# OpenDriveLab/kai0

Measured on AMD Instinct MI355X. Metric: train samples/sec pi0.5 full FT, higher is better.
Workload: dtype bf16; 1 GPU; pi0.5 full fine-tune bf16, batch 32 per MI355X, 3-cam 224x224 (BASELINE.json configs[1]); global_batch=32, seq_len=1018, parallelism=dp1

## Files before the change

### kai0_amd/csrc/gemm_bf16.hip

```cpp
#include "common.h"
#include "../../include/kai0hip.h"
#include <stdlib.h>
#include <algorithm>
#include <atomic>
#include <type_traits>

namespace {

constexpr int BK = 64;

#ifdef KAI0_ABLATE
#define KAI0_ABL(p) ((p).ablate)
#else
#define KAI0_ABL(p) 0
#endif

struct RowMap {
    int32_t rpb;
    int64_t bs, off;
    __device__ __forceinline__ int64_t operator()(int r) const {
        if (rpb == 0) return r;
        const int q = r / rpb;
        return (int64_t)q * bs + (r - q * rpb) + off;
    }
};

struct GemmArgs {
    const bf16_t* A;
    const bf16_t* B;
    void* C;
    int M, N, K;
    int64_t lda, ldb, ldc;
    int batch_inner;
    int64_t sA1, sA2, sB1, sB2, sC1, sC2;
    RowMap amap, bmap, cmap;
    const void* bias;
    int bias_f32;
    float scale;
    int act;
    int out_f32;
    bf16_t* pre_out;
    const bf16_t* aux1;
    const bf16_t* aux2;
    const bf16_t* gate;
    int gate_rpb;
    int accumulate;
    int64_t gate_ld;
    const bf16_t* residual;
    int64_t ldr, sR1, sR2;
    int tiles_m, tiles_n;
    int ablate;
    int nt_c;
    int simple_epi;
    int nt_pre;
    const float* rowvec;
    int64_t rv_s1, rv_s2, rv_ld;
    int nseg;
    bf16_t* seg_dst[3];
    int64_t seg_ld[3];
    int seg_begin[3];
    float* ws;
    int split_k, k_chunk;
    const bf16_t* B2;
    bf16_t* pre_out2;
    bf16_t* norm_out;
    const void* norm_w;
    const bf16_t* norm_b;
    float norm_eps;
    int norm_kind;
    const bf16_t* rope_cos;
    const bf16_t* rope_sin;
    int rope_half, rope_n_end;
};

typedef __attribute__((ext_vector_type(4))) int i32x4_t;
constexpr uint32_t OOB = 0x80000000u;
__device__ __forceinline__ void glds16(__amdgpu_buffer_rsrc_t rsrc, uint32_t voff, char* lds_dst_wave_uniform) {
    __builtin_amdgcn_raw_ptr_buffer_load_lds(rsrc, (LDS_PTR(void))lds_dst_wave_uniform, 16, (int)voff, 0, 0, 0);
}


__device__ __forceinline__ void store_pre8(bf16_t* dst, bf16x8 v, int nt) {
    if (nt) __builtin_nontemporal_store(v, reinterpret_cast<bf16x8*>(dst));
    else *reinterpret_cast<bf16x8*>(dst) = v;
}

// ... 99 lines not shown
        }
        *reinterpret_cast<f32x4*>(cp) = f32x4{v[0], v[1], v[2], v[3]};
        *reinterpret_cast<f32x4*>(cp + 4) = f32x4{v[4], v[5], v[6], v[7]};
    } else {
        bf16_t* cp = reinterpret_cast<bf16_t*>(cbase) + cz + orow * p.ldc + ccol;
        if (p.nseg > 0) {
            int si = 0;
            if (p.nseg > 1 && ccol >= p.seg_begin[1]) si = 1;
            if (p.nseg > 2 && ccol >= p.seg_begin[2]) si = 2;
            cp = p.seg_dst[si] + orow * p.seg_ld[si] + (ccol - p.seg_begin[si]);
        }
        if (p.accumulate) {
            bf16x8 ov = *reinterpret_cast<const bf16x8*>(cp);
#pragma unroll
            for (int e = 0; e < 8; ++e) v[e] += bf2f(ov[e]);
        }
        bf16x8 ov;
#pragma unroll
        for (int e = 0; e < 8; ++e) ov[e] = f2bf(v[e]);
        store_pre8(cp, ov, p.nt_c);
    }
}

#define N_ALIGNED8(n) (((n) & 7) == 0)

__device__ __forceinline__ void lds_barrier() {
    __builtin_amdgcn_sched_barrier(0);
    asm volatile("s_waitcnt lgkmcnt(0)" ::: "memory");
    __builtin_amdgcn_s_barrier();
    asm volatile("" ::: "memory");
    __builtin_amdgcn_sched_barrier(0);
}

template <bool A_KC, bool B_KC, int WM, int WN, int MT, int NT, bool PP, int NS = 2, int BKT = 64, int SCH = 0>
__global__ __launch_bounds__(WM * WN * 64, (WM * WN * 64) / 256) void gemm_bf16_kernel(const GemmArgs p) {
    static_assert(PP ? (WM == 2 && WN == 4 && MT == 8 && ((SCH == 1 && NS == 2 && BKT == 64) || (SCH == 3 && NS == 4 && BKT == 32)))
                     : (SCH == 0 && NS >= 2 && BKT == 64),
                  "K loops: plain multi-stage (SCH 0, 64 deep), quadrant (SCH 1: 256x256x64, 2 stages), ring (SCH 3: 256x256x32, 4 slots)");
    constexpr int BK = BKT;
    constexpr int NWAVES = WM * WN;
    constexpr int TBM = WM * MT * 16, TBN = WN * NT * 16;
    constexpr int A_TILE = TBM * BK * 2, B_TILE = TBN * BK * 2;
    constexpr int STAGE = A_TILE + B_TILE;
    constexpr int NA = A_TILE / 1024 / NWAVES;
    constexpr int NB = B_TILE / 1024 / NWAVES;
    constexpr int KC_CPR = BK / 8;
    constexpr int KC_RPP = 64 / KC_CPR;
    constexpr int A_ROWB = TBM * 2, B_ROWB = TBN * 2;
    constexpr int A_LPR = A_ROWB / 16, B_LPR = B_ROWB / 16;
    constexpr int A_RPP = 64 / A_LPR, B_RPP = 64 / B_LPR;
    constexpr int GROUP = TBM == 128 ? 8 : 4;
    static_assert(NA >= 1 && NB >= 1 && NT == 4 && ((MT % 4) == 0 || MT == 2), "unsupported tile configuration");
    constexpr int AH = MT >= 4 ? 4 : MT;
    static_assert(A_KC || (64 % A_LPR) == 0, "contraction-strided A needs a power-of-two tile height");
    extern __shared__ __attribute__((aligned(16))) char smem[];

    const int tid = threadIdx.x;
    const int lane = tid & 63;
    const int wave = __builtin_amdgcn_readfirstlane(tid >> 6);
    const int wm = wave / WN, wn = wave % WN;
    if constexpr (MT <= 4) {
        asm volatile("" ::"s"(p.A), "s"(p.B), "s"(p.M), "s"(p.N), "s"(p.K), "s"(p.lda), "s"(p.ldb), "s"(p.tiles_m), "s"(p.tiles_n),
                     "s"(p.split_k), "s"(p.k_chunk), "s"(p.batch_inner), "s"(p.amap.rpb), "s"(p.bmap.rpb), "s"(p.act), "s"(p.sA1),
                     "s"(p.sB1), "s"(p.sA2), "s"(p.sB2));
    }
    const int nwg = gridDim.x;
    int pid = blockIdx.x;
    {
// ... 252 lines not shown
        issue_half(false, 1, 0);
        issue_half(false, 0, 1);
        issue_half(true, 1, 1);
        asm volatile("s_waitcnt vmcnt(6)" ::: "memory");
        lds_barrier();
        if (grp == 1) lds_barrier();
        bf16x8 af[4][2], bq[2][2];
        auto read_a = [&](const char* ta, int h) {
#pragma unroll
            for (int i = 0; i < 4; ++i)
#pragma unroll
                for (int ks = 0; ks < 2; ++ks)
                    af[i][ks] = A_KC ? load_frag(ta, true, A_ROWB, wm * 128 + (h * 4 + i) * 16, ks)
                                     : load_frag(ta + h * 16384, false, 256, wm * 64 + i * 16, ks);
        };
        auto read_b = [&](const char* tb, int h) {
#pragma unroll
            for (int j = 0; j < 2; ++j)
#pragma unroll
                for (int ks = 0; ks < 2; ++ks)
                    bq[j][ks] = B_KC ? load_frag(tb, true, B_ROWB, wn * 64 + (h * 2 + j) * 16, ks)
                                     : load_frag(tb + h * 16384, false, 256, wn * 32 + j * 16, ks);
        };
        auto quad = [&](auto ahc, auto bhc) {
            constexpr int ah = decltype(ahc)::value, bh = decltype(bhc)::value;
            __builtin_amdgcn_s_setprio(1);
#pragma unroll
            for (int ks = 0; ks < 2; ++ks)
#pragma unroll
                for (int i = 0; i < 4; ++i)
#pragma unroll
                    for (int j = 0; j < 2; ++j)
                        acc[ah * 4 + i][bh * 2 + j] =
                            __builtin_amdgcn_mfma_f32_16x16x32_bf16(af[i][ks], bq[j][ks], acc[ah * 4 + i][bh * 2 + j], 0, 0, 0);
            __builtin_amdgcn_s_setprio(0);
        };
        using I0 = std::integral_constant<int, 0>;
        using I1 = std::integral_constant<int, 1>;
        for (int t = 0; t < nk; ++t) {
            const char* ta = smem + (t & 1) * STAGE;
            const char* tb = ta + A_TILE;
            read_b(tb, 0);
            __builtin_amdgcn_sched_barrier(0);
            read_a(ta, 0);
            __builtin_amdgcn_sched_barrier(0);
            issue_half(true, 0, t + 1);
            lds_barrier();
            quad(I0{}, I0{});
            lds_barrier();
            read_b(tb, 1);
            __builtin_amdgcn_sched_barrier(0);
            issue_half(false, 1, t + 1);
            asm volatile("s_waitcnt vmcnt(8)" ::: "memory");
            lds_barrier();
            quad(I0{}, I1{});
            lds_barrier();
            read_a(ta, 1);
            __builtin_amdgcn_sched_barrier(0);
            issue_half(false, 0, t + 2);
            lds_barrier();
            quad(I1{}, I1{});
            lds_barrier();
            read_b(tb, 0);
            __builtin_amdgcn_sched_barrier(0);
            issue_half(true, 1, t + 2);
            asm volatile("s_waitcnt vmcnt(6)" ::: "memory");
            lds_barrier();
            quad(I1{}, I0{});
            lds_barrier();
        }
        asm volatile("s_waitcnt vmcnt(0)" ::: "memory");
        if (grp == 0) lds_barrier();
        lds_barrier();
    } else {
#pragma unroll
        for (int st = 0; st < NS - 1; ++st)
            if (st < nk) stage(st, st);
        int slot_c = 0, slot_p = NS - 1;
        for (int kt = 0; kt < nk; ++kt) {
            if constexpr (NS == 2) {
                asm volatile("s_waitcnt vmcnt(0)" ::: "memory");
            } else {
                if (kt + NS - 2 < nk) asm volatile("s_waitcnt vmcnt(%0)" ::"n"((NS - 2) * (NA + NB)) : "memory");
                else asm volatile("s_waitcnt vmcnt(0)" ::: "memory");
            }
            lds_barrier();
            if (kt + NS - 1 < nk && KAI0_ABL(p) != 1) stage(kt + NS - 1, slot_p);
            const char* ta = smem + slot_c * STAGE;
            const char* tb = ta + A_TILE;
    #pragma unroll
            for (int ks = 0; ks < BK / 32; ++ks) {
                bf16x8 bfr[NT];
    #pragma unroll
                for (int t = 0; t < NT; ++t) bfr[t] = load_frag(tb, B_KC, B_ROWB, wn * (NT * 16) + t * 16, ks);
    #pragma unroll
                for (int h = 0; h < MT / AH; ++h) {
                    bf16x8 af[AH];
    #pragma unroll
                    for (int t = 0; t < AH; ++t) af[t] = load_frag(ta, A_KC, A_ROWB, wm * (MT * 16) + (h * AH + t) * 16, ks);
    #pragma unroll
                    for (int i = 0; i < AH; ++i)
    #pragma unroll
                        for (int j = 0; j < NT; ++j)
                            acc[h * AH + i][j] = __builtin_amdgcn_mfma_f32_16x16x32_bf16(af[i], bfr[j], acc[h * AH + i][j], 0, 0, 0);
                }
            }
            slot_c = slot_c + 1 == NS ? 0 : slot_c + 1;
            slot_p = slot_p + 1 == NS ? 0 : slot_p + 1;
        }
        lds_barrier();
    }

    float* slab = reinterpret_cast<float*>(smem + wave * (AH * 4096));
    const int64_t cz = z1 * p.sC1 + z2 * p.sC2;
    const int64_t rz = z1 * p.sR1 + z2 * p.sR2;
    const int64_t vz = z1 * p.rv_s1 + z2 * p.rv_s2;
    constexpr bool ILM = SCH == 1 && !A_KC, ILN = SCH == 1 && !B_KC;
    const int ccol = ILN ? n0 + ((lane & 7) >> 2) * 128 + wn * 32 + ((lane & 7) & 3) * 8 : n0 + wn * 64 + (lane & 7) * 8;
    auto row_base = [&](int h) { return ILM ? m0 + h * 128 + wm * 64 : m0 + wm * (MT * 16) + h * 64; };
    const bool col_ok = ccol < ((p.N + 7) & ~7);
    const bool fused_fast = p.act >= 2 && p.split_k == 1 && p.bias == nullptr && p.gate == nullptr && p.residual == nullptr &&
                            !p.accumulate && !p.out_f32 && p.nseg == 0 && (p.act == 4 || p.scale == 1.0f) &&
                            (p.act != 3 || p.pre_out != nullptr);
    const bool plain_fast = p.act <= 1 && p.split_k == 1 && (p.bias != nullptr || p.residual != nullptr) && p.gate == nullptr &&
                            !p.accumulate && !p.out_f32 && p.nseg == 0 && (N_ALIGNED8(p.N));
    const bool simple_fast = MT == 8 && p.simple_epi && p.act <= 1 && p.split_k == 1 && p.gate == nullptr && !p.out_f32 && p.scale == 1.0f &&
                             p.cmap.rpb == 0 && (N_ALIGNED8(p.N));
    auto epi_half = [&](auto hc) {
        constexpr int h = decltype(hc)::value;
        if constexpr (((MT == 4 && WM == 2) || (MT == 2 && WM == 4)) && WN == 2 && A_KC && B_KC) if (p.act == 7) {
            const bool rot = n0 < p.rope_n_end;
            const int fi = ((n0 >> 7) & 1) * 64 + (lane & 7) * 8;
            const int rcol = rot ? (n0 >> 8) * 256 + wn * 128 + fi : n0 + wn * 64 + (lane & 7) * 8;
            const int rbase = row_base(h) + (lane >> 3);
            bf16x8 cs[AH * 2], sn[AH * 2];
#pragma unroll
            for (int it = 0; it < AH * 2; ++it) {
                const int64_t tr = (int64_t)min(rbase + it * 8, p.M - 1) * p.rope_half + fi;
                cs[it] = *reinterpret_cast<const bf16x8*>(p.rope_cos + (rot ? tr : 0));
                sn[it] = *reinterpret_cast<const bf16x8*>(p.rope_sin + (rot ? tr : 0));
            }
#pragma unroll
            for (int i = 0; i < AH; ++i)
#pragma unroll
                for (int j = 0; j < 4; ++j)
#pragma unroll
                    for (int r = 0; r < 4; ++r) slab[(i * 16 + 4 * g + r) * 64 + j * 16 + l15] = acc[i][j][r];
            lds_barrier();
            const float* pslab = reinterpret_cast<const float*>(smem + (wave ^ 1) * (AH * 4096));
            int si = 0;
            if (p.nseg > 1 && rcol >= p.seg_begin[1]) si = 1;
            if (p.nseg > 2 && rcol >= p.seg_begin[2]) si = 2;
            const bool rcol_ok = rcol < p.N;
#pragma unroll
            for (int it = 0; it < AH * 2; ++it) {
                const int lr = it * 8 + (lane >> 3);
                const int row = rbase + it * 8;
                const int so = lr * 64 + (lane & 7) * 8;
                const f32x4 v0 = *reinterpret_cast<const f32x4*>(slab + so), v1 = *reinterpret_cast<const f32x4*>(slab + so + 4);
                const f32x4 w0 = *reinterpret_cast<const f32x4*>(pslab + so), w1 = *reinterpret_cast<const f32x4*>(pslab + so + 4);
// ... 334 lines not shown
            float v[8] = {v0[0], v0[1], v0[2], v0[3], v1[0], v1[1], v1[2], v1[3]};
            if (p.split_k > 1) {
                float* wp = reinterpret_cast<float*>(p.ws) + ((int64_t)blockIdx.y * p.M + row) * p.N + ccol;
                *reinterpret_cast<f32x4*>(wp) = v0;
                *reinterpret_cast<f32x4*>(wp + 4) = v1;
            } else {
                epilogue8(p, v, row, ccol, cz, rz, vz, p.C, p.out_f32 != 0);
            }
        }
        asm volatile("s_waitcnt lgkmcnt(0)" ::: "memory");
        __builtin_amdgcn_wave_barrier();
    };
    epi_half(std::integral_constant<int, 0>{});
    if constexpr (MT / 4 > 1) epi_half(std::integral_constant<int, 1>{});
    if constexpr (MT / 4 > 2) epi_half(std::integral_constant<int, 2>{});
    static_assert(MT / 4 <= 3, "extend the epilogue parts");
}

constexpr int PS_SLOTS = 1024;
__device__ unsigned int g_ps_ctr[PS_SLOTS][16];

#ifdef KAI0_PS_TRACE
__device__ long long g_ps_trace[256][8];
#define PS_STAMP(i)                                              \
    do {                                                         \
        const long long n_ = __builtin_amdgcn_s_memrealtime();   \
        t_acc[i] += n_ - t_prev;                                 \
        t_prev = n_;                                             \
    } while (0)
#else
#define PS_STAMP(i) do { } while (0)
#endif

__global__ __launch_bounds__(512, 1) void gemm_nt_persistent_kernel(const GemmArgs p, unsigned int* __restrict__ ctr) {
    constexpr int TBM = 256, TBN = 256, A_TILE = TBM * BK * 2, STAGE = 2 * A_TILE, GROUP = 4, MT = 8;
    extern __shared__ __attribute__((aligned(16))) char smem[];
    const int tid = threadIdx.x, lane = tid & 63;
    const int wave = __builtin_amdgcn_readfirstlane(tid >> 6);
    const int wm = wave >> 2, wn = wave & 3, grp = wm;
    const int l15 = lane & 15, g = lane >> 4;
    int* mbox = reinterpret_cast<int*>(smem + 2 * STAGE);
    float* slab = reinterpret_cast<float*>(smem + 2 * STAGE + wave * 4096);
    const int ntile = p.tiles_m * p.tiles_n;
    const int qq = ntile >> 3, rr = ntile & 7;
    const int x0 = blockIdx.x & 7;
    auto draw = [&]() -> unsigned { return __hip_atomic_fetch_add(ctr + x0, 1u, __ATOMIC_RELAXED, __HIP_MEMORY_SCOPE_AGENT); };
    auto resolve = [&](unsigned t) -> int {
        for (int a = 0; a < 8; ++a) {
            const int x = (x0 + a) & 7;
            const int len = qq + (x < rr ? 1 : 0);
            if (a > 0) t = __hip_atomic_fetch_add(ctr + x, 1u, __ATOMIC_RELAXED, __HIP_MEMORY_SCOPE_AGENT);
            if ((int)t < len) return (x < rr ? x * (qq + 1) : rr * (qq + 1) + (x - rr) * qq) + (int)t;
        }
        return -1;
    };
    auto next_ticket = [&]() -> int { return resolve(draw()); };
    const __amdgpu_buffer_rsrc_t a_rsrc = __builtin_amdgcn_make_buffer_rsrc((void*)p.A, 0, (int)OOB, 0x00020000);
    const __amdgpu_buffer_rsrc_t b_rsrc = __builtin_amdgcn_make_buffer_rsrc((void*)p.B, 0, (int)OOB, 0x00020000);
    const bool pair = p.act == 6;
    const __amdgpu_buffer_rsrc_t b2_rsrc = __builtin_amdgcn_make_buffer_rsrc((void*)(pair ? p.B2 : p.B), 0, (int)OOB, 0x00020000);
    const int kc_chunk = ((lane & 7) ^ (lane >> 3)) * 8;
    const int nk = (p.K + BK - 1) / BK;

    const uint32_t lda2 = (uint32_t)p.lda * 2, ldb2 = (uint32_t)p.ldb * 2, kc2 = (uint32_t)kc_chunk * 2;
    auto arow_fix = [](int) -> uint32_t { return 0u; };
    int m0 = 0, n0 = 0;
// ... 74 lines not shown
#ifdef KAI0_PS_TRACE
    long long t_acc[5] = {0, 0, 0, 0, 0};
    long long t_prev = __builtin_amdgcn_s_memrealtime();
#endif
    while (cur >= 0) {
        f32x4 acc[MT][4];
#pragma unroll
        for (int i = 0; i < MT; ++i)
#pragma unroll
            for (int j = 0; j < 4; ++j) acc[i][j] = f32x4{0.f, 0.f, 0.f, 0.f};
        bf16x8 af[4][2], bq[2][2];
        auto read_a = [&](const char* ta, int h) {
#pragma unroll
            for (int i = 0; i < 4; ++i)
#pragma unroll
                for (int ks = 0; ks < 2; ++ks) af[i][ks] = frag(ta, wm * 128 + (h * 4 + i) * 16, ks);
        };
        auto read_b = [&](const char* tb, int h) {
#pragma unroll
            for (int j = 0; j < 2; ++j)
#pragma unroll
                for (int ks = 0; ks < 2; ++ks) bq[j][ks] = frag(tb, wn * 64 + (h * 2 + j) * 16, ks);
        };
        auto quad = [&](auto ahc, auto bhc) {
            constexpr int ah = decltype(ahc)::value, bh = decltype(bhc)::value;
            __builtin_amdgcn_s_setprio(1);
#pragma unroll
            for (int ks = 0; ks < 2; ++ks)
#pragma unroll
                for (int i = 0; i < 4; ++i)
#pragma unroll
                    for (int j = 0; j < 2; ++j)
                        acc[ah * 4 + i][bh * 2 + j] =
                            __builtin_amdgcn_mfma_f32_16x16x32_bf16(af[i][ks], bq[j][ks], acc[ah * 4 + i][bh * 2 + j], 0, 0, 0);
            __builtin_amdgcn_s_setprio(0);
        };
        using I0 = std::integral_constant<int, 0>;
        using I1 = std::integral_constant<int, 1>;
        PS_STAMP(0);
        for (int t = 0; t < nk; ++t) {
            const char* ta = smem + (t & 1) * STAGE;
            const char* tb = ta + A_TILE;
            read_b(tb, 0);
            __builtin_amdgcn_sched_barrier(0);
            read_a(ta, 0);
            __builtin_amdgcn_sched_barrier(0);
            issue_half(true, 0, t + 1);
            lds_barrier();
            quad(I0{}, I0{});
            lds_barrier();
            read_b(tb, 1);
            __builtin_amdgcn_sched_barrier(0);
            issue_half(false, 1, t + 1);
            asm volatile("s_waitcnt vmcnt(8)" ::: "memory");
            lds_barrier();
            quad(I0{}, I1{});
            lds_barrier();
            read_a(ta, 1);
            __builtin_amdgcn_sched_barrier(0);
            issue_half(false, 0, t + 2);
            lds_barrier();
            quad(I1{}, I1{});
            lds_barrier();
            read_b(tb, 0);
            __builtin_amdgcn_sched_barrier(0);
            issue_half(true, 1, t + 2);
            asm volatile("s_waitcnt vmcnt(6)" ::: "memory");
            lds_barrier();
            quad(I1{}, I0{});
            lds_barrier();
        }
        asm volatile("s_waitcnt vmcnt(0)" ::: "memory");
        if (grp == 0) lds_barrier();
        lds_barrier();

        PS_STAMP(1);
        const int m0c = m0, n0c = n0;
        int nn = -1;
        unsigned raw = 0;
        if (tid == 0 && nxt >= 0) raw = draw();
        if (nxt >= 0) {
            setup(nxt);
            prologue_issue();
        }
        const int ccol = n0c + wn * 64 + (lane & 7) * 8;
        const bool col_ok = ccol < ((p.N + 7) & ~7);
        const bool fused_fast = p.act >= 2 && p.act <= 5 && p.bias == nullptr && p.gate == nullptr && p.residual == nullptr && !p.accumulate &&
                                !p.out_f32 && p.nseg == 0 && (p.act == 4 || p.scale == 1.0f) && (p.act != 3 || p.pre_out != nullptr);
        const bool simple_fast = p.simple_epi && p.act <= 1 && p.split_k == 1 && p.gate == nullptr && !p.out_f32 && p.scale == 1.0f && p.cmap.rpb == 0 &&
                                 (N_ALIGNED8(p.N));
        auto to_slab = [&](int ti) {
            __builtin_amdgcn_wave_barrier();
#pragma unroll
            for (int j = 0; j < 4; ++j)
#pragma unroll
                for (int r = 0; r < 4; ++r) slab[(4 * g + r) * 64 + j * 16 + l15] = acc[ti][j][r];
            asm volatile("s_waitcnt lgkmcnt(0)" ::: "memory");
            __builtin_amdgcn_wave_barrier();
        };
        if (pair) {
            const int ocol = (n0c >> 1) + wn * 32 + (lane & 3) * 8;
            const bool ocol_ok = ocol < (p.N >> 1);
            bf16_t* cb = reinterpret_cast<bf16_t*>(p.C);
#pragma unroll
            for (int ti = 0; ti < MT; ++ti) {
                to_slab(ti);
                const int row = m0c + wm * 128 + ti * 16 + (lane >> 2);
                const float* sp = slab + (lane >> 2) * 64 + (lane & 3) * 8;
                const f32x4 g0 = *reinterpret_cast<const f32x4*>(sp), g1 = *reinterpret_cast<const f32x4*>(sp + 4);
                const f32x4 u0 = *reinterpret_cast<const f32x4*>(sp + 32), u1 = *reinterpret_cast<const f32x4*>(sp + 36);
                if (row < p.M && ocol_ok) {
                    const float gv[8] = {g0[0], g0[1], g0[2], g0[3], g1[0], g1[1], g1[2], g1[3]};
                    const float uv[8] = {u0[0], u0[1], u0[2], u0[3], u1[0], u1[1], u1[2], u1[3]};
                    bf16x8 gb, ub, hb;
#pragma unroll
                    for (int e = 0; e < 8; e += 2) {
                        const f32x2 gr = rbf2(f32x2{gv[e], gv[e + 1]}), ur = rbf2(f32x2{uv[e], uv[e + 1]});
                        const f32x2 hv = rbf2(gelu_tanh2(gr)) * ur;
                        gb[e] = f2bf(gr[0]); gb[e + 1] = f2bf(gr[1]);
                        ub[e] = f2bf(ur[0]); ub[e + 1] = f2bf(ur[1]);
                        hb[e] = f2bf(hv[0]); hb[e + 1] = f2bf(hv[1]);
                    }
                    const int64_t o = p.cmap(row) * p.ldc + ocol;
                    *reinterpret_cast<bf16x8*>(cb + o) = hb;
                    if (p.pre_out != nullptr) store_pre8(p.pre_out + o, gb, p.nt_pre);
                    if (p.pre_out2 != nullptr) store_pre8(p.pre_out2 + o, ub, p.nt_pre);
                }
            }
        } else if (fused_fast) {
            bf16_t* cb = reinterpret_cast<bf16_t*>(p.C);
#pragma unroll
            for (int h = 0; h < 2; ++h) {
                bf16x8 s0[8], s1[8];
// ... 300 lines not shown
        float ss = 0.f;
#pragma unroll
        for (int e = 0; e < 8; ++e) ss += x[e] * x[e];
        const float rstd = rsqrtf(block_sum<4>(ss, red) / (float)p.N + p.norm_eps);
#pragma unroll
        for (int e = 0; e < 8; ++e) y[e] = (x[e] * rstd) * (1.0f + wv[e]);
    } else {
        float sm = 0.f;
#pragma unroll
        for (int e = 0; e < 8; ++e) sm += x[e];
        const float mean = block_sum<4>(sm, red) / (float)p.N;
        float vs = 0.f;
#pragma unroll
        for (int e = 0; e < 8; ++e) {
            const float d = x[e] - mean;
            vs += live ? d * d : 0.f;
        }
        const float rstd = rsqrtf(block_sum<4>(vs, red) / (float)p.N + p.norm_eps);
#pragma unroll
        for (int e = 0; e < 8; ++e) y[e] = (x[e] - mean) * rstd * wv[e] + bv[e];
    }
    if (live) {
        bf16x8 o;
#pragma unroll
        for (int e = 0; e < 8; ++e) o[e] = f2bf(y[e]);
        *reinterpret_cast<bf16x8*>(p.norm_out + (int64_t)row * p.N + col) = o;
    }
}

constexpr int layout_bit(bool a_kc, bool b_kc) { return 1 << (2 * a_kc + b_kc); }
constexpr int L_NT = layout_bit(true, true), L_NN = layout_bit(true, false), L_TT = layout_bit(false, true), L_TN = layout_bit(false, false);
constexpr int L_ALL = L_NT | L_NN | L_TT | L_TN;

template <int LAYOUTS, int WM, int WN, int MT, int NT, bool PP, int NS = 2, int BKT = 64, int SCH = 0>
int launch_cfg(const kai0_gemm_desc* d, GemmArgs& p, int batch, hipStream_t s) {
    constexpr int TBM = WM * MT * 16, TBN = WN * NT * 16;
    constexpr int LDS = NS * (TBM + TBN) * BKT * 2;
    p.tiles_m = (d->M + TBM - 1) / TBM;
    p.tiles_n = (p.N + TBN - 1) / TBN;
    dim3 grid(p.tiles_m * p.tiles_n, batch * p.split_k, 1), block(WM * WN * 64, 1, 1);
#define KAI0_LAUNCH(AK, BK_)                                                                                      \
    if constexpr ((LAYOUTS & layout_bit(AK, BK_)) != 0)                                                          \
        if ((d->a_kc != 0) == AK && (d->b_kc != 0) == BK_) {                                                      \
            static bool attr_set = false;                                                                         \
            auto kern = gemm_bf16_kernel<AK, BK_, WM, WN, MT, NT, PP, NS, BKT, SCH>;                              \
            if (!attr_set) {                                                                                      \
                hipError_t e = hipFuncSetAttribute((const void*)kern, hipFuncAttributeMaxDynamicSharedMemorySize, LDS); \
                if (e != hipSuccess) {                                                                            \
                    kai0_set_error("kai0_gemm_bf16: cannot reserve %d B of LDS: %s", LDS, hipGetErrorString(e));  \
                    return -2;                                                                                    \
                }                                                                                                 \
                attr_set = true;                                                                                  \
            }                                                                                                     \
            hipLaunchKernelGGL(kern, grid, block, LDS, s, p);                                                     \
            return 0;                                                                                             \
        }
    KAI0_LAUNCH(true, true)
    KAI0_LAUNCH(true, false)
    KAI0_LAUNCH(false, true)
    KAI0_LAUNCH(false, false)
#undef KAI0_LAUNCH
    kai0_set_error("kai0_gemm_bf16: the %d x %d tile configuration (%d waves, %d stages) is not built for a_kc=%d b_kc=%d", TBM, TBN,
                   WM * WN, NS, d->a_kc, d->b_kc);
    return -3;
}

}

#ifdef KAI0_PS_TRACE
KAI0_API int kai0_debug_ps_trace(long long* host_out) {
    return (int)hipMemcpyFromSymbol(host_out, HIP_SYMBOL(g_ps_trace), sizeof(long long) * 256 * 8);
}
#endif

KAI0_API int kai0_gemm_bf16(const kai0_gemm_desc* d, kai0_stream_t stream) {
    KAI0_REQUIRE(d != nullptr, "kai0_gemm_bf16: null descriptor");
    KAI0_REQUIRE(d->M > 0 && d->N > 0 && d->K > 0, "kai0_gemm_bf16: empty problem M=%d N=%d K=%d", d->M, d->N,
                 d->K);
    KAI0_REQUIRE(d->A && d->B && d->C, "kai0_gemm_bf16: null operand");
    KAI0_REQUIRE((d->lda % 8) == 0 && (d->ldb % 8) == 0 && (d->ldc % 8) == 0,
                 "kai0_gemm_bf16: leading dims must be multiples of 8 (lda=%lld ldb=%lld ldc=%lld)",
                 (long long)d->lda, (long long)d->ldb, (long long)d->ldc);
    KAI0_REQUIRE((d->N % 8) == 0 || (d->b_kc && d->ldc >= ((d->N + 7) & ~7) && !d->bias && !d->gate && !d->residual &&
                                     !d->pre_out && !d->accumulate),
                 "kai0_gemm_bf16: N=%d not a multiple of 8 needs b_kc, padded C rows and a plain epilogue", d->N);
    KAI0_REQUIRE((d->K % 8) == 0 || (!d->a_kc && !d->b_kc), "kai0_gemm_bf16: K=%d must be a multiple of 8 for "
                 "K-contiguous operands", d->K);
    KAI0_REQUIRE(d->a_kc || (d->M % 8) == 0, "kai0_gemm_bf16: M=%d must be a multiple of 8 when A is [K][M]",
                 d->M);
    KAI0_REQUIRE(((uintptr_t)d->A % 16) == 0 && ((uintptr_t)d->B % 16) == 0 && ((uintptr_t)d->C % 16) == 0,
                 "kai0_gemm_bf16: operands must be 16-byte aligned");
    KAI0_REQUIRE(d->batch <= 1 || (((d->sA1 | d->sA2 | d->sB1 | d->sB2) & 7) == 0 && ((d->sC1 | d->sC2) & (d->out_f32 ? 3 : 7)) == 0),
                 "kai0_gemm_bf16: batch strides must be multiples of 8 elements (16 B)");
    KAI0_REQUIRE(d->gate == nullptr || d->gate_rpb > 0, "kai0_gemm_bf16: gate needs gate_rpb > 0");
    KAI0_REQUIRE(d->act >= 0 && d->act <= 7, "kai0_gemm_bf16: unknown act %d", d->act);
    KAI0_REQUIRE(d->persist >= 0 && d->persist <= 2 && d->small_w8 >= 0 && d->small_w8 <= 2 && d->general_epilogue >= 0 &&
                     d->general_epilogue <= 1,
                 "kai0_gemm_bf16: hook out of range (persist=%d, small_w8=%d: 0..2; general_epilogue=%d: 0..1)", d->persist, d->small_w8,
                 d->general_epilogue);
    KAI0_REQUIRE(d->act != 7 || (d->rope_cos && d->rope_sin && d->rope_half == 128 && d->rope_n_end > 0 && (d->rope_n_end % 256) == 0 &&
                                 d->rope_n_end <= d->N && (d->N % 128) == 0 && d->a_kc && d->b_kc && d->batch <= 1 && d->split_k <= 1 &&
                                 !d->out_f32 && !d->accumulate && !d->bias && !d->gate && !d->residual && !d->pre_out &&
                                 (d->scale == 0.0f || d->scale == 1.0f) && d->b_rpb == 0 && ((uintptr_t)d->rope_cos % 16) == 0 &&
                                 ((uintptr_t)d->rope_sin % 16) == 0),
                 "kai0_gemm_bf16: act=7 (RoPE epilogue) needs bf16 cos / sin tables [M][128], rope_n_end %% 256 == 0, N %% 128 == 0, K-contiguous "
                 "operands, one batch entry, no split-K, a plain bf16 output");
    KAI0_REQUIRE(d->act != 6 || (d->B2 && d->a_kc && d->b_kc && d->batch <= 1 && d->split_k <= 1 && !d->out_f32 && !d->accumulate &&
                                 d->nseg == 0 && !d->bias && !d->gate && !d->residual && (d->scale == 0.0f || d->scale == 1.0f) &&
                                 (d->N % 32) == 0 && d->b_rpb == 0 && ((uintptr_t)d->B2 % 16) == 0),
                 "kai0_gemm_bf16: act=6 (GeGLU pair) needs B2 = up weight, K-contiguous operands, N %% 32 == 0, one batch entry, a "
                 "plain bf16 output");
    KAI0_REQUIRE(d->norm_kind == 0 ||
                     ((d->norm_kind == 1 || d->norm_kind == 2) && d->split_k > 1 && d->norm_out && d->norm_w && (d->norm_kind == 1 || d->norm_b) &&
                      d->batch <= 1 && !d->out_f32 && d->nseg == 0 && (d->N % 8) == 0 && d->N <= 2048 && d->act == 0 && !d->gate &&
                      !d->rowvec && ((uintptr_t)d->norm_out % 16) == 0 && ((uintptr_t)d->norm_w % 16) == 0),
                 "kai0_gemm_bf16: a fused norm (norm_kind=%d) needs split_k > 1, norm_out / norm_w (/ norm_b), one batch entry, a plain "
                 "bf16 output with N %% 8 == 0, N <= 2048, no activation / gate", d->norm_kind);
    KAI0_REQUIRE(d->act != 5 || (d->aux1 && !d->out_f32 && !d->accumulate && d->nseg == 0 && (d->N % 8) == 0),
                 "kai0_gemm_bf16: act=5 (fused GELU backward) needs aux1 = pre-activation, plain bf16 output");
    KAI0_REQUIRE(d->act != 4 || (d->aux1 && d->rowvec && !d->out_f32 && !d->accumulate && d->nseg == 0 && (d->N % 8) == 0),
                 "kai0_gemm_bf16: act=4 (fused softmax backward) needs aux1 = P, rowvec = D, plain bf16 output");
    KAI0_REQUIRE(d->act < 2 || d->act >= 4 || ((d->pre_out || d->act == 2) && d->aux1 && (d->act == 2 || d->aux2) && !d->out_f32 && (d->N % 8) == 0),
                 "kai0_gemm_bf16: act=%d (fused GeGLU) needs pre_out and aux inputs, bf16 output", d->act);
    KAI0_REQUIRE(d->nseg >= 0 && d->nseg <= 3, "kai0_gemm_bf16: nseg=%d", d->nseg);
    if (d->nseg > 0) {
        KAI0_REQUIRE(!d->out_f32 && !d->accumulate && (d->batch <= 1) && (d->act < 2 || d->act == 7) && !d->pre_out && (d->N % 8) == 0,
                     "kai0_gemm_bf16: column segments need a plain bf16 epilogue, batch 1");
        KAI0_REQUIRE(d->act != 4, "kai0_gemm_bf16: column segments and act=4 are exclusive");
        for (int i = 0; i < d->nseg; ++i)
            KAI0_REQUIRE(d->seg[i].dst && (d->seg[i].ld % 8) == 0 && (d->seg[i].n_begin % 8) == 0 &&
                             ((uintptr_t)d->seg[i].dst % 16) == 0 && d->seg[i].n_begin == (i ? d->seg[i].n_begin : 0) &&
// ... 19 lines not shown
    p.pre_out2 = (bf16_t*)d->pre_out2;
    p.norm_out = (bf16_t*)d->norm_out;
    p.norm_w = d->norm_w;
    p.norm_b = (const bf16_t*)d->norm_b;
    p.norm_eps = d->norm_eps;
    p.norm_kind = d->norm_kind;
    p.rope_cos = (const bf16_t*)d->rope_cos;
    p.rope_sin = (const bf16_t*)d->rope_sin;
    p.rope_half = d->rope_half;
    p.rope_n_end = d->rope_n_end;
    p.lda = d->lda; p.ldb = d->ldb; p.ldc = d->ldc;
    p.batch_inner = d->batch_inner > 0 ? d->batch_inner : 1;
    p.sA1 = d->sA1; p.sA2 = d->sA2; p.sB1 = d->sB1; p.sB2 = d->sB2; p.sC1 = d->sC1; p.sC2 = d->sC2;
    p.amap = RowMap{d->a_rpb, d->a_bs, d->a_off};
    p.bmap = RowMap{d->b_rpb, d->b_bs, d->b_off};
    p.cmap = RowMap{d->c_rpb, d->c_bs, d->c_off};
    p.bias = d->bias; p.bias_f32 = d->bias_f32;
    p.scale = d->scale == 0.0f ? 1.0f : d->scale;
    p.act = d->act; p.out_f32 = d->out_f32;
    p.pre_out = (bf16_t*)d->pre_out;
    p.aux1 = (const bf16_t*)d->aux1;
    p.aux2 = (const bf16_t*)d->aux2;
    p.gate = (const bf16_t*)d->gate; p.gate_rpb = d->gate_rpb; p.gate_ld = d->gate_ld;
    p.accumulate = d->accumulate;
    p.residual = (const bf16_t*)d->residual; p.ldr = d->ldr; p.sR1 = d->sR1; p.sR2 = d->sR2;
#ifdef KAI0_ABLATE
    static const int ablate = [] { const char* e = getenv("KAI0_GEMM_ABLATE"); return e ? atoi(e) : 0; }();
    p.ablate = ablate;
#else
    p.ablate = 0;
#endif
    p.nt_pre = 1;
    p.nt_c = d->c_nontemporal != 0;
    p.simple_epi = d->general_epilogue == 0;
    p.rowvec = d->rowvec; p.rv_s1 = d->rv_s1; p.rv_s2 = d->rv_s2; p.rv_ld = d->rv_ld;
    p.nseg = d->nseg;
    for (int i = 0; i < 3; ++i) {
        p.seg_dst[i] = i < d->nseg ? (bf16_t*)d->seg[i].dst : nullptr;
        p.seg_ld[i] = i < d->nseg ? d->seg[i].ld : 0;
        p.seg_begin[i] = i < d->nseg ? d->seg[i].n_begin : 0;
    }
    p.split_k = 1;
    p.k_chunk = d->K;
    const int split = d->split_k > 1 ? d->split_k : 1;
    p.ws = nullptr;
    if (split > 1) {
        KAI0_REQUIRE(d->workspace != nullptr && d->workspace_bytes >= (int64_t)batch * split * d->M * d->N * 4,
                     "kai0_gemm_bf16: split_k=%d needs a workspace of batch*split*M*N*4 bytes", split);
        KAI0_REQUIRE((d->N % 8) == 0, "kai0_gemm_bf16: split_k needs N %% 8 == 0");
        p.split_k = split;
        p.k_chunk = ((d->K + split - 1) / split + BK - 1) / BK * BK;
        p.ws = (float*)d->workspace;
    }
    const int64_t big_tiles = (int64_t)((d->M + 255) / 256) * ((p.N + 255) / 256) * batch * (split > 1 ? split : 1);
    const bool big = d->act != 7 && big_tiles >= 160 && d->K >= 256;
    hipStream_t s = (hipStream_t)stream;
    int rc;
    const int64_t small_blocks = (int64_t)((d->M + 127) / 128) * ((p.N + 127) / 128) * batch * (split > 1 ? split : 1);
    const bool deep = small_blocks <= 256 && p.k_chunk >= 256;
    const bool w8 = !big && d->a_kc && d->b_kc && (d->act <= 1 || d->act == 7) && (d->small_w8 == 2 || (d->small_w8 == 0 && deep));
    const int persist = d->persist == 1 ? 0 : (d->persist == 2 ? 2 : 1);
    const bool ps_ok = persist && big && d->a_kc && d->b_kc && batch == 1 && split == 1 &&
                       big_tiles >= (persist == 2 ? 512 : 2048) &&
                       (p.K % 8) == 0 && !d->rowvec && d->a_rpb == 0 && d->b_rpb == 0;
    const bool ps_rule = p.N >= 8192 || d->K >= 8192;
    if (ps_ok && (persist == 2 || ps_rule)) {
        constexpr int LDS = 2 * 2 * 256 * 64 * 2 + 8 * 4096;
        struct PsDev { unsigned int* ctr = nullptr; int cus = 0; };
        static PsDev ps_dev[64];
        static std::atomic<unsigned> next_slot{0};
        int dv = 0;
        KAI0_REQUIRE(hipGetDevice(&dv) == hipSuccess && dv >= 0 && dv < 64, "kai0_gemm_bf16: hipGetDevice");
        PsDev& pd = ps_dev[dv];
        if (pd.ctr == nullptr) {
            void* sym = nullptr;
            hipError_t e = hipGetSymbolAddress(&sym, HIP_SYMBOL(g_ps_ctr));
            if (e == hipSuccess) e = hipFuncSetAttribute((const void*)gemm_nt_persistent_kernel, hipFuncAttributeMaxDynamicSharedMemorySize, LDS);
            hipDeviceProp_t pr;
            if (e == hipSuccess) e = hipGetDeviceProperties(&pr, dv);
            KAI0_REQUIRE(e == hipSuccess, "kai0_gemm_bf16: persistent kernel setup failed: %s", hipGetErrorString(e));
            pd.cus = pr.multiProcessorCount > 0 ? pr.multiProcessorCount : 256;
            pd.ctr = (unsigned int*)sym;
        }
        unsigned int* ctr_base = pd.ctr;
        p.tiles_m = (d->M + 255) / 256;
        p.tiles_n = (p.N + 255) / 256;
        const int nblk = (int)std::min<int64_t>(big_tiles, pd.cus);
        unsigned int* ctr = ctr_base + (size_t)(next_slot.fetch_add(1) % PS_SLOTS) * 16;
        hipLaunchKernelGGL(gemm_nt_persistent_kernel, dim3(nblk), dim3(512), LDS, s, p, ctr);
        return kai0_check_launch("kai0_gemm_bf16 (persistent)");
    }
    if (big && d->a_kc && d->b_kc) rc = launch_cfg<L_NT, 2, 4, 8, 4, true, 2, 64, 1>(d, p, batch, s);
    else if (big && !d->a_kc && !d->b_kc) rc = launch_cfg<L_TN, 2, 4, 8, 4, true, 4, 32, 3>(d, p, batch, s);
    else if (big) rc = launch_cfg<L_NN | L_TT, 2, 4, 8, 4, false>(d, p, batch, s);
    else if (w8) rc = launch_cfg<L_NT, 4, 2, 2, 4, false, 4>(d, p, batch, s);
    else if (deep) rc = launch_cfg<L_ALL, 2, 2, 4, 4, false, 4>(d, p, batch, s);
    else rc = launch_cfg<L_ALL, 2, 2, 4, 4, false>(d, p, batch, s);
    if (rc) return rc;
    rc = kai0_check_launch("kai0_gemm_bf16");
    if (rc || split == 1) return rc;
    if (d->norm_kind != 0) {
        if (d->norm_kind == 1) hipLaunchKernelGGL(splitk_reduce_norm_kernel<1>, dim3(d->M), dim3(256), 0, s, p);
        else hipLaunchKernelGGL(splitk_reduce_norm_kernel<2>, dim3(d->M), dim3(256), 0, s, p);
        return kai0_check_launch("kai0_gemm_bf16(split-K reduce + norm)");
    }
    const int64_t items = (int64_t)d->M * (d->N / 8);
    int rb = (int)((items + 255) / 256);
    if (rb > 2048) rb = 2048;
    hipLaunchKernelGGL(splitk_reduce_kernel, dim3(rb, batch, 1), dim3(256), 0, s, p);
    return kai0_check_launch("kai0_gemm_bf16(split-K reduce)");
}
```

Measured before the change: 68.74 samples/s.

## Add direct-store epilogue for big NT GEMMs using swapped MFMA and lane permutes

For large NT GEMMs with simple epilogues (bias, GELU, residual, accumulate), the MFMA operands are swapped so each lane holds accumulator values along columns. The values are then transposed across lanes with permlane swaps and stored straight to global memory as 8-wide bf16 vectors. This skips the LDS slab staging round trip and the final barriers in the quadrant and persistent kernels. It adds a new template variant and uses bf16 rounding before GELU, which changes numerics slightly. Each store row is a 16-byte write, which may coalesce less well than the slab path.

```diff
diff --git a/kai0_amd/csrc/gemm_bf16.hip b/kai0_amd/csrc/gemm_bf16.hip
--- a/kai0_amd/csrc/gemm_bf16.hip
+++ b/kai0_amd/csrc/gemm_bf16.hip
@@ -51,7 +51,7 @@
     int tiles_m, tiles_n;
     int ablate;
     int nt_c;
-    int simple_epi;
+    int epi_path;
     int nt_pre;
     const float* rowvec;
     int64_t rv_s1, rv_s2, rv_ld;
@@ -217,8 +217,144 @@
     __builtin_amdgcn_sched_barrier(0);
 }
 
-template <bool A_KC, bool B_KC, int WM, int WN, int MT, int NT, bool PP, int NS = 2, int BKT = 64, int SCH = 0>
+__device__ __forceinline__ uint32_t pack_bf2(float a, float b) {
+    return __builtin_bit_cast(uint32_t, __builtin_convertvector(f32x2{a, b}, bf16x2_t));
+}
+__device__ __forceinline__ void xchg16(uint32_t& a, uint32_t& b) {
+    const auto s = __builtin_amdgcn_permlane16_swap(a, b, false, false);
+    a = s[0];
+    b = s[1];
+}
+__device__ __forceinline__ void xchg32(uint32_t& a, uint32_t& b) {
+    const auto s = __builtin_amdgcn_permlane32_swap(a, b, false, false);
+    a = s[0];
+    b = s[1];
+}
+__device__ __forceinline__ void transpose4(uint32_t (&x)[4]) {
+    xchg32(x[0], x[2]);
+    xchg32(x[1], x[3]);
+    xchg16(x[0], x[1]);
+    xchg16(x[2], x[3]);
+}
+
+__device__ __forceinline__ void direct_simple_epilogue(const GemmArgs& p, const f32x4 (&acc)[8][4], int row0, int col0, int64_t cz,
+                                                       int64_t rz, int lane) {
+    const int l15 = lane & 15, g = lane >> 4;
+    const bool has_bias = p.bias != nullptr, has_res = p.residual != nullptr, gelu = p.act == 1, accum = p.accumulate != 0;
+    const int M_ = p.M, N_ = p.N, nt_pre_ = p.nt_pre, nt_c_ = p.nt_c;
+    const bf16_t* res_ = p.residual;
+    bf16_t* pre_ = p.pre_out;
+    const int64_t ldr_ = p.ldr, ldc_ = p.ldc;
+    float bv[4][4];
+#pragma unroll
+    for (int j = 0; j < 4; ++j) {
+        const int c = col0 + j * 16 + 4 * g;
+        f32x4 b = f32x4{0.f, 0.f, 0.f, 0.f};
+        if (has_bias && c < N_) {
+            if (p.bias_f32) {
+                b = *reinterpret_cast<const f32x4*>(reinterpret_cast<const float*>(p.bias) + c);
+            } else {
+                const bf16x4 b4 = *reinterpret_cast<const bf16x4*>(reinterpret_cast<const bf16_t*>(p.bias) + c);
+                b = f32x4{bf2f(b4[0]), bf2f(b4[1]), bf2f(b4[2]), bf2f(b4[3])};
+            }
+        }
+#pragma unroll
+        for (int r = 0; r < 4; ++r) bv[j][r] = b[r];
+    }
+    int cc[2];
+    bool ok[2];
+    bf16_t* cl[2];
+    int64_t ldl[2];
+#pragma unroll
+    for (int q = 0; q < 2; ++q) {
+        const int ccol = col0 + g * 16 + q * 8;
+        cc[q] = ccol;
+        ok[q] = ccol < N_;
+        cl[q] = reinterpret_cast<bf16_t*>(p.C) + cz + ccol;
+        ldl[q] = p.ldc;
+        if (p.nseg > 0) {
+            cl[q] = p.seg_dst[0] + (ccol - p.seg_begin[0]);
+            ldl[q] = p.seg_ld[0];
+            if (p.nseg > 1 && ccol >= p.seg_begin[1]) {
+                cl[q] = p.seg_dst[1] + (ccol - p.seg_begin[1]);
+                ldl[q] = p.seg_ld[1];
+            }
+            if (p.nseg > 2 && ccol >= p.seg_begin[2]) {
+                cl[q] = p.seg_dst[2] + (ccol - p.seg_begin[2]);
+                ldl[q] = p.seg_ld[2];
+            }
+        }
+    }
+    const int rbase = row0 + l15;
+    auto res_row = [&](int i, int q) -> bf16x8 {
+        const int row = rbase + i * 16;
+        return (has_res && row < M_ && ok[q]) ? *reinterpret_cast<const bf16x8*>(res_ + rz + (int64_t)row * ldr_ + cc[q]) : bf16x8{};
+    };
+    auto old_row = [&](int i, int q) -> bf16x8 {
+        const int row = rbase + i * 16;
+        return (accum && row < M_ && ok[q]) ? *reinterpret_cast<const bf16x8*>(cl[q] + (int64_t)row * ldl[q]) : bf16x8{};
+    };
+    bf16x8 rnext[2] = {res_row(0, 0), res_row(0, 1)}, onext[2] = {old_row(0, 0), old_row(0, 1)};
+#pragma unroll
+    for (int i = 0; i < 8; ++i) {
+        const int row = rbase + i * 16;
+        uint32_t x0[4], x1[4];
+#pragma unroll
+        for (int j = 0; j < 4; ++j) {
+            f32x4 v = acc[i][j];
+            if (has_bias) {
+#pragma unroll
+                for (int r = 0; r < 4; ++r) v[r] += bv[j][r];
+            }
+            x0[j] = pack_bf2(v[0], v[1]);
+            x1[j] = pack_bf2(v[2], v[3]);
+        }
+        transpose4(x0);
+        transpose4(x1);
+        const bf16x8 rv[2] = {rnext[0], rnext[1]}, ov0[2] = {onext[0], onext[1]};
+        if (i + 1 < 8) {
+#pragma unroll
+            for (int q = 0; q < 2; ++q) {
+                rnext[q] = res_row(i + 1, q);
+                onext[q] = old_row(i + 1, q);
+            }
+        }
+#pragma unroll
+        for (int q = 0; q < 2; ++q) {
+            bf16x8 o = __builtin_bit_cast(bf16x8, u32x4{x0[2 * q], x1[2 * q], x0[2 * q + 1], x1[2 * q + 1]});
+            if (row >= M_ || !ok[q]) continue;
+            if (gelu || has_res || accum) {
+                float v[8];
+#pragma unroll
+                for (int e = 0; e < 8; ++e) v[e] = bf2f(o[e]);
+                if (gelu) {
+                    if (pre_ != nullptr) store_pre8(pre_ + cz + (int64_t)row * ldc_ + cc[q], o, nt_pre_);
+#pragma unroll
+                    for (int e = 0; e < 8; e += 2) {
+                        const f32x2 a = gelu_tanh2(f32x2{v[e], v[e + 1]});
+                        v[e] = rbf(a[0]);
+                        v[e + 1] = rbf(a[1]);
+                    }
+                }
+                if (has_res) {
+#pragma unroll
+                    for (int e = 0; e < 8; ++e) v[e] = rbf(v[e] + bf2f(rv[q][e]));
+                }
+                if (accum) {
+#pragma unroll
+                    for (int e = 0; e < 8; ++e) v[e] += bf2f(ov0[q][e]);
+                }
+#pragma unroll
+                for (int e = 0; e < 8; ++e) o[e] = f2bf(v[e]);
+            }
+            store_pre8(cl[q] + (int64_t)row * ldl[q], o, nt_c_);
+        }
+    }
+}
+
+template <bool A_KC, bool B_KC, int WM, int WN, int MT, int NT, bool PP, int NS = 2, int BKT = 64, int SCH = 0, bool DIR = false>
 __global__ __launch_bounds__(WM * WN * 64, (WM * WN * 64) / 256) void gemm_bf16_kernel(const GemmArgs p) {
+    static_assert(!DIR || (SCH == 1 && A_KC && B_KC), "direct-store epilogue: NT quadrant configuration only");
     static_assert(PP ? (WM == 2 && WN == 4 && MT == 8 && ((SCH == 1 && NS == 2 && BKT == 64) || (SCH == 3 && NS == 4 && BKT == 32)))
                      : (SCH == 0 && NS >= 2 && BKT == 64),
                   "K loops: plain multi-stage (SCH 0, 64 deep), quadrant (SCH 1: 256x256x64, 2 stages), ring (SCH 3: 256x256x32, 4 slots)");
@@ -537,7 +673,8 @@
 #pragma unroll
                     for (int j = 0; j < 2; ++j)
                         acc[ah * 4 + i][bh * 2 + j] =
-                            __builtin_amdgcn_mfma_f32_16x16x32_bf16(af[i][ks], bq[j][ks], acc[ah * 4 + i][bh * 2 + j], 0, 0, 0);
+                            DIR ? __builtin_amdgcn_mfma_f32_16x16x32_bf16(bq[j][ks], af[i][ks], acc[ah * 4 + i][bh * 2 + j], 0, 0, 0)
+                                : __builtin_amdgcn_mfma_f32_16x16x32_bf16(af[i][ks], bq[j][ks], acc[ah * 4 + i][bh * 2 + j], 0, 0, 0);
             __builtin_amdgcn_s_setprio(0);
         };
         using I0 = std::integral_constant<int, 0>;
@@ -574,9 +711,9 @@
             quad(I1{}, I0{});
             lds_barrier();
         }
-        asm volatile("s_waitcnt vmcnt(0)" ::: "memory");
+        if constexpr (!DIR) asm volatile("s_waitcnt vmcnt(0)" ::: "memory");
         if (grp == 0) lds_barrier();
-        lds_barrier();
+        if constexpr (!DIR) lds_barrier();
     } else {
 #pragma unroll
         for (int st = 0; st < NS - 1; ++st)
@@ -616,9 +753,13 @@
         lds_barrier();
     }
 
-    float* slab = reinterpret_cast<float*>(smem + wave * (AH * 4096));
     const int64_t cz = z1 * p.sC1 + z2 * p.sC2;
     const int64_t rz = z1 * p.sR1 + z2 * p.sR2;
+    if constexpr (DIR) {
+        direct_simple_epilogue(p, acc, m0 + wm * 128, n0 + wn * 64, cz, rz, lane);
+        return;
+    }
+    float* slab = reinterpret_cast<float*>(smem + wave * (AH * 4096));
     const int64_t vz = z1 * p.rv_s1 + z2 * p.rv_s2;
     constexpr bool ILM = SCH == 1 && !A_KC, ILN = SCH == 1 && !B_KC;
     const int ccol = ILN ? n0 + ((lane & 7) >> 2) * 128 + wn * 32 + ((lane & 7) & 3) * 8 : n0 + wn * 64 + (lane & 7) * 8;
@@ -629,8 +770,7 @@
                             (p.act != 3 || p.pre_out != nullptr);
     const bool plain_fast = p.act <= 1 && p.split_k == 1 && (p.bias != nullptr || p.residual != nullptr) && p.gate == nullptr &&
                             !p.accumulate && !p.out_f32 && p.nseg == 0 && (N_ALIGNED8(p.N));
-    const bool simple_fast = MT == 8 && p.simple_epi && p.act <= 1 && p.split_k == 1 && p.gate == nullptr && !p.out_f32 && p.scale == 1.0f &&
-                             p.cmap.rpb == 0 && (N_ALIGNED8(p.N));
+    const bool simple_fast = MT == 8 && p.epi_path == 1;
     auto epi_half = [&](auto hc) {
         constexpr int h = decltype(hc)::value;
         if constexpr (((MT == 4 && WM == 2) || (MT == 2 && WM == 4)) && WN == 2 && A_KC && B_KC) if (p.act == 7) {
@@ -1031,6 +1171,7 @@
 #define PS_STAMP(i) do { } while (0)
 #endif
 
+template <bool DIR>
 __global__ __launch_bounds__(512, 1) void gemm_nt_persistent_kernel(const GemmArgs p, unsigned int* __restrict__ ctr) {
     constexpr int TBM = 256, TBN = 256, A_TILE = TBM * BK * 2, STAGE = 2 * A_TILE, GROUP = 4, MT = 8;
     extern __shared__ __attribute__((aligned(16))) char smem[];
@@ -1171,7 +1312,8 @@
 #pragma unroll
                     for (int j = 0; j < 2; ++j)
                         acc[ah * 4 + i][bh * 2 + j] =
-                            __builtin_amdgcn_mfma_f32_16x16x32_bf16(af[i][ks], bq[j][ks], acc[ah * 4 + i][bh * 2 + j], 0, 0, 0);
+                            DIR ? __builtin_amdgcn_mfma_f32_16x16x32_bf16(bq[j][ks], af[i][ks], acc[ah * 4 + i][bh * 2 + j], 0, 0, 0)
+                                : __builtin_amdgcn_mfma_f32_16x16x32_bf16(af[i][ks], bq[j][ks], acc[ah * 4 + i][bh * 2 + j], 0, 0, 0);
             __builtin_amdgcn_s_setprio(0);
         };
         using I0 = std::integral_constant<int, 0>;
@@ -1226,8 +1368,7 @@
         const bool col_ok = ccol < ((p.N + 7) & ~7);
         const bool fused_fast = p.act >= 2 && p.act <= 5 && p.bias == nullptr && p.gate == nullptr && p.residual == nullptr && !p.accumulate &&
                                 !p.out_f32 && p.nseg == 0 && (p.act == 4 || p.scale == 1.0f) && (p.act != 3 || p.pre_out != nullptr);
-        const bool simple_fast = p.simple_epi && p.act <= 1 && p.split_k == 1 && p.gate == nullptr && !p.out_f32 && p.scale == 1.0f && p.cmap.rpb == 0 &&
-                                 (N_ALIGNED8(p.N));
+        const bool simple_fast = p.epi_path == 1;
         auto to_slab = [&](int ti) {
             __builtin_amdgcn_wave_barrier();
 #pragma unroll
@@ -1237,7 +1378,10 @@
             asm volatile("s_waitcnt lgkmcnt(0)" ::: "memory");
             __builtin_amdgcn_wave_barrier();
         };
-        if (pair) {
+        if constexpr (DIR) {
+            direct_simple_epilogue(p, acc, m0c + wm * 128, n0c + wn * 64, cz, rz, lane);
+            __builtin_amdgcn_s_waitcnt(0x0F70);
+        } else if (pair) {
             const int ocol = (n0c >> 1) + wn * 32 + (lane & 3) * 8;
             const bool ocol_ok = ocol < (p.N >> 1);
             bf16_t* cb = reinterpret_cast<bf16_t*>(p.C);
@@ -1604,7 +1748,7 @@
 constexpr int L_NT = layout_bit(true, true), L_NN = layout_bit(true, false), L_TT = layout_bit(false, true), L_TN = layout_bit(false, false);
 constexpr int L_ALL = L_NT | L_NN | L_TT | L_TN;
 
-template <int LAYOUTS, int WM, int WN, int MT, int NT, bool PP, int NS = 2, int BKT = 64, int SCH = 0>
+template <int LAYOUTS, int WM, int WN, int MT, int NT, bool PP, int NS = 2, int BKT = 64, int SCH = 0, bool DIR = false>
 int launch_cfg(const kai0_gemm_desc* d, GemmArgs& p, int batch, hipStream_t s) {
     constexpr int TBM = WM * MT * 16, TBN = WN * NT * 16;
     constexpr int LDS = NS * (TBM + TBN) * BKT * 2;
@@ -1615,7 +1759,7 @@
     if constexpr ((LAYOUTS & layout_bit(AK, BK_)) != 0)                                                          \
         if ((d->a_kc != 0) == AK && (d->b_kc != 0) == BK_) {                                                      \
             static bool attr_set = false;                                                                         \
-            auto kern = gemm_bf16_kernel<AK, BK_, WM, WN, MT, NT, PP, NS, BKT, SCH>;                              \
+            auto kern = gemm_bf16_kernel<AK, BK_, WM, WN, MT, NT, PP, NS, BKT, SCH, DIR>;                         \
             if (!attr_set) {                                                                                      \
                 hipError_t e = hipFuncSetAttribute((const void*)kern, hipFuncAttributeMaxDynamicSharedMemorySize, LDS); \
                 if (e != hipSuccess) {                                                                            \
@@ -1667,8 +1811,8 @@
     KAI0_REQUIRE(d->gate == nullptr || d->gate_rpb > 0, "kai0_gemm_bf16: gate needs gate_rpb > 0");
     KAI0_REQUIRE(d->act >= 0 && d->act <= 7, "kai0_gemm_bf16: unknown act %d", d->act);
     KAI0_REQUIRE(d->persist >= 0 && d->persist <= 2 && d->small_w8 >= 0 && d->small_w8 <= 2 && d->general_epilogue >= 0 &&
-                     d->general_epilogue <= 1,
-                 "kai0_gemm_bf16: hook out of range (persist=%d, small_w8=%d: 0..2; general_epilogue=%d: 0..1)", d->persist, d->small_w8,
+                     d->general_epilogue <= 2,
+                 "kai0_gemm_bf16: hook out of range (persist=%d, small_w8=%d, general_epilogue=%d: 0..2)", d->persist, d->small_w8,
                  d->general_epilogue);
     KAI0_REQUIRE(d->act != 7 || (d->rope_cos && d->rope_sin && d->rope_half == 128 && d->rope_n_end > 0 && (d->rope_n_end % 256) == 0 &&
                                  d->rope_n_end <= d->N && (d->N % 128) == 0 && d->a_kc && d->b_kc && d->batch <= 1 && d->split_k <= 1 &&
@@ -1754,7 +1898,6 @@
 #endif
     p.nt_pre = 1;
     p.nt_c = d->c_nontemporal != 0;
-    p.simple_epi = d->general_epilogue == 0;
     p.rowvec = d->rowvec; p.rv_s1 = d->rv_s1; p.rv_s2 = d->rv_s2; p.rv_ld = d->rv_ld;
     p.nseg = d->nseg;
     for (int i = 0; i < 3; ++i) {
@@ -1776,6 +1919,11 @@
     }
     const int64_t big_tiles = (int64_t)((d->M + 255) / 256) * ((p.N + 255) / 256) * batch * (split > 1 ? split : 1);
     const bool big = d->act != 7 && big_tiles >= 160 && d->K >= 256;
+    const bool simple_ok = d->general_epilogue != 1 && d->act <= 1 && split == 1 && !d->gate && !d->out_f32 && p.scale == 1.0f &&
+                           d->c_rpb == 0 && (p.N % 8) == 0;
+    const bool nt_big = big && d->a_kc && d->b_kc;
+    const bool direct_simple = d->general_epilogue == 0 && simple_ok && nt_big;
+    p.epi_path = direct_simple ? 2 : (simple_ok ? 1 : 0);
     hipStream_t s = (hipStream_t)stream;
     int rc;
     const int64_t small_blocks = (int64_t)((d->M + 127) / 128) * ((p.N + 127) / 128) * batch * (split > 1 ? split : 1);
@@ -1797,7 +1945,8 @@
         if (pd.ctr == nullptr) {
             void* sym = nullptr;
             hipError_t e = hipGetSymbolAddress(&sym, HIP_SYMBOL(g_ps_ctr));
-            if (e == hipSuccess) e = hipFuncSetAttribute((const void*)gemm_nt_persistent_kernel, hipFuncAttributeMaxDynamicSharedMemorySize, LDS);
+            if (e == hipSuccess) e = hipFuncSetAttribute((const void*)gemm_nt_persistent_kernel<false>, hipFuncAttributeMaxDynamicSharedMemorySize, LDS);
+            if (e == hipSuccess) e = hipFuncSetAttribute((const void*)gemm_nt_persistent_kernel<true>, hipFuncAttributeMaxDynamicSharedMemorySize, LDS);
             hipDeviceProp_t pr;
             if (e == hipSuccess) e = hipGetDeviceProperties(&pr, dv);
             KAI0_REQUIRE(e == hipSuccess, "kai0_gemm_bf16: persistent kernel setup failed: %s", hipGetErrorString(e));
@@ -1809,10 +1958,12 @@
         p.tiles_n = (p.N + 255) / 256;
         const int nblk = (int)std::min<int64_t>(big_tiles, pd.cus);
         unsigned int* ctr = ctr_base + (size_t)(next_slot.fetch_add(1) % PS_SLOTS) * 16;
-        hipLaunchKernelGGL(gemm_nt_persistent_kernel, dim3(nblk), dim3(512), LDS, s, p, ctr);
+        if (p.epi_path == 2) hipLaunchKernelGGL(gemm_nt_persistent_kernel<true>, dim3(nblk), dim3(512), LDS, s, p, ctr);
+        else hipLaunchKernelGGL(gemm_nt_persistent_kernel<false>, dim3(nblk), dim3(512), LDS, s, p, ctr);
         return kai0_check_launch("kai0_gemm_bf16 (persistent)");
     }
-    if (big && d->a_kc && d->b_kc) rc = launch_cfg<L_NT, 2, 4, 8, 4, true, 2, 64, 1>(d, p, batch, s);
+    if (nt_big && p.epi_path == 2) rc = launch_cfg<L_NT, 2, 4, 8, 4, true, 2, 64, 1, true>(d, p, batch, s);
+    else if (nt_big) rc = launch_cfg<L_NT, 2, 4, 8, 4, true, 2, 64, 1>(d, p, batch, s);
     else if (big && !d->a_kc && !d->b_kc) rc = launch_cfg<L_TN, 2, 4, 8, 4, true, 4, 32, 3>(d, p, batch, s);
     else if (big) rc = launch_cfg<L_NN | L_TT, 2, 4, 8, 4, false>(d, p, batch, s);
     else if (w8) rc = launch_cfg<L_NT, 4, 2, 2, 4, false, 4>(d, p, batch, s);
```

Measured after the change: 68.29 samples/s. No clear change (-0.7%).
